# arkworks-rs/poly-commit

Measured on AMD Instinct MI355X. Metric: MSM G1-scalar-pairs/sec inside KZG commit+open (MarlinKZG10<Bls12_381> shape, hiding off), inputs HBM-resident (host-input blocking calls: value_trait_shaped), higher is better.
Workload: dtype u32 limbs (381-bit Fq / 255-bit Fr modular integer); 1 GPU; MarlinKZG10<bls12_381> commit+open, dense poly deg 2^24 per GPU, true SRS resident, hiding off (BASELINE metric sizes: 2^20 = configs[1], 2^24 = north-star target); curve=bls12_381, log_degree=24, inflight=2, srs_window_table=True, parallelism=1 GPU

## Files before the change

### __graft_entry__.py

```python
import os
import subprocess
import sys

ROOT = os.path.dirname(os.path.abspath(__file__))
for p in (ROOT, os.path.join(ROOT, "tests"), os.path.join(ROOT, "oracle")):
    if p not in sys.path:
        sys.path.insert(0, p)


def build():
    import importlib
    b = importlib.import_module("poly_commit_amd.build")
    b.build()
    subprocess.check_call(["make", "-s", "-C", os.path.join(ROOT, "oracle")])
    mb = os.path.join(ROOT, "tools", "microbench")
    src = mb + ".hip"
    deps = [src] + [os.path.join(ROOT, "poly_commit_amd", "csrc", f) for f in ("ec.hpp", "fp32.hpp", "curves.hpp")]
    deps = [d for d in deps if os.path.exists(d)]
    if not os.path.exists(mb) or any(os.path.getmtime(d) > os.path.getmtime(mb) for d in deps):
        subprocess.check_call(["hipcc", "--offload-arch=gfx950", "-O3", "-std=c++17", "-w", "-o", mb, src])
    import poly_commit_amd as pc
    pc.load_library()


def smoke():
    import numpy as np
    import oracle_lib as O
    import poly_commit_amd as pc

    if not os.path.exists(pc.library_path()):
        raise RuntimeError("libpc_hip.so missing -- run build() first (no CPU fallback exists)")
    ctx = pc.Context(0)
    curve, d = "bls12_381", 1 << 10
    powers = O.gen_bases(curve, d + 1)
    coeffs = O.f_to_mont(curve, 1, O.gen_scalars(curve, 0x5EED0001, d + 1))
    z = O.f_to_mont(curve, 1, O.gen_scalars(curve, 7, 1))[0]
    srs = ctx.upload_srs(curve, powers)
    comm, _ = srs.msm(coeffs, montgomery=True)
    q = ctx.witness_poly(curve, coeffs, z)
    proof, _ = srs.msm(q, montgomery=True)
    rc1, want_c = O.kzg_commit(curve, powers, coeffs)
    rc2, want_w = O.kzg_open(curve, powers, coeffs, z)
    assert rc1 == 0 and rc2 == 0
    assert (comm == want_c).all(), "commitment differs from the oracle"
    assert (proof == want_w).all(), "opening proof differs from the oracle"
    srs.precompute(min_pairs=1)
    assert (srs.msm(coeffs, montgomery=True)[0] == want_c).all(), "commitment (window table) differs from the oracle"
    assert (srs.msm(q, montgomery=True)[0] == want_w).all(), "opening proof (window table) differs from the oracle"
    rows = np.ascontiguousarray(coeffs[:1024].reshape(32, 32, 4))
    can = O.f_from_mont(curve, 1, np.ascontiguousarray(coeffs[:1024])).reshape(32, 32, 4)
    many, _ = srs.msm_many(rows, montgomery=True)
    for k in (0, 17, 31):
        assert (many[k] == O.msm_naive(curve, powers[:32], np.ascontiguousarray(can[k]))).all(), "msm_many differs from the oracle"
    mat = coeffs[:1024].reshape(4, 256, 4)
    assert (ctx.ntt_batch(curve, mat, 10) == O.ntt_batch(curve, mat, 10)).all(), "NTT differs from the oracle"
    srs.free()
    ctx.close()
    print("smoke ok: commit, open (table-free and window table), msm_many and NTT bit-identical to the oracle")


if __name__ == "__main__":
    build()
    if len(sys.argv) > 1 and sys.argv[1] == "smoke":
        smoke()
```

### poly_commit_amd/csrc/ec.hpp

```cpp
#pragma once
#include "fp32.hpp"

namespace pc {

template <class C>
struct AffD {
  typedef Fd<typename C::FqP> Fq;
  Fq x, y;
  static PC_HD AffD infinity() { AffD a; a.x = Fq::zero(); a.y = Fq::zero(); return a; }
  PC_HD bool is_inf() const { return x.is_zero() && y.is_zero(); }
  static PC_HD AffD load(const uint32_t* p) { AffD a; a.x = Fq::load(p); a.y = Fq::load(p + Fq::N); return a; }
  PC_HD void store(uint32_t* p) const { x.store(p); y.store(p + Fq::N); }
  PC_HD AffD neg_if(bool s) const { AffD a; a.x = x; a.y = s ? y.neg() : y; return a; }
};

template <class C>
struct XyzzD {
  typedef Fd<typename C::FqP> Fq;
  static constexpr int WORDS = 4 * Fq::N;
  Fq X, Y, ZZ, ZZZ;

  static PC_HD XyzzD infinity() { XyzzD r; r.X = Fq::zero(); r.Y = Fq::zero(); r.ZZ = Fq::zero(); r.ZZZ = Fq::zero(); return r; }
  PC_HD bool is_inf() const { return ZZ.is_zero(); }
  static PC_HD XyzzD from_affine(const AffD<C>& a) {
    XyzzD r;
    if (a.is_inf()) return infinity();
    r.X = a.x; r.Y = a.y; r.ZZ = Fq::one(); r.ZZZ = Fq::one(); return r;
  }
  static PC_HD XyzzD load(const uint32_t* p) {
    XyzzD r; r.X = Fq::load(p); r.Y = Fq::load(p + Fq::N); r.ZZ = Fq::load(p + 2 * Fq::N); r.ZZZ = Fq::load(p + 3 * Fq::N); return r;
  }
  PC_HD void store(uint32_t* p) const { X.store(p); Y.store(p + Fq::N); ZZ.store(p + 2 * Fq::N); ZZZ.store(p + 3 * Fq::N); }

  static PC_HD XyzzD dbl_affine(const AffD<C>& a) {
    if (a.is_inf() || a.y.is_zero()) return infinity();
    XyzzD r;
    Fq U = a.y.dbl(), V = U.sqr(), W = U.mul(V), S = a.x.mul(V);
    Fq xx = a.x.sqr(), M = xx.dbl().add(xx);
    r.X = M.sqr().sub(S.dbl());
    r.Y = M.mul_add_mul(S.sub(r.X), W.neg(), a.y);
    r.ZZ = V; r.ZZZ = W;
    return r;
  }
  PC_HD XyzzD dbl() const {
    if (is_inf() || Y.is_zero()) return infinity();
    XyzzD r;
    Fq U = Y.dbl(), V = U.sqr(), W = U.mul(V), S = X.mul(V);
    Fq xx = X.sqr(), M = xx.dbl().add(xx);
    r.X = M.sqr().sub(S.dbl());
    r.Y = M.mul_add_mul(S.sub(r.X), W.neg(), Y);
    r.ZZ = V.mul(ZZ); r.ZZZ = W.mul(ZZZ);
    return r;
  }
  PC_HD void add_affine(const AffD<C>& a) {
    if (a.is_inf()) return;
    if (is_inf()) { X = a.x; Y = a.y; ZZ = Fq::one(); ZZZ = Fq::one(); return; }
    Fq U2 = a.x.mul(ZZ), S2 = a.y.mul(ZZZ);
    Fq Pp = U2.sub(X), R = S2.sub(Y);
    if (Pp.is_zero()) {
      if (R.is_zero()) *this = dbl_affine(a); else *this = infinity();
      return;
    }
    Fq PP = Pp.sqr(), PPP = Pp.mul(PP), Q = X.mul(PP);
    Fq X3 = R.sqr().sub(PPP).sub(Q.dbl());
    Y = R.mul_add_mul(Q.sub(X3), Y.neg(), PPP);
    X = X3;
    ZZ = ZZ.mul(PP); ZZZ = ZZZ.mul(PPP);
  }
  PC_HD void add_affine_lz(const AffD<C>& a, bool negate) {
    if (a.y.is_zero()) { if (a.x.is_zero()) return; }
    const Fq ay = negate ? a.y.neg_lz_canonical() : a.y;
    if (is_inf()) { X = a.x; Y = ay; ZZ = Fq::one(); ZZZ = Fq::one(); return; }
    Fq U2 = a.x.mul_lz(ZZ), S2 = ay.mul_lz(ZZZ);
    Fq Pp = U2.sub_lz(X), R = S2.sub_lz(Y);
    if (Pp.is_zero_lz()) {
      XyzzD t = canonical();
      AffD<C> b; b.x = a.x; b.y = ay.canon();
      t.add_affine(b);
      *this = t;
      return;
    }
    Fq PP = Pp.sqr_lz(), PPP = Pp.mul_lz(PP), Q = X.mul_lz(PP);
    Fq X3 = R.sqr_lz().sub_lz(PPP).sub_lz(Q.dbl_lz());
    Y = R.mul_add_mul_lz(Q.sub_lz(X3), Y.neg_lz(), PPP);
    X = X3;
    ZZ = ZZ.mul_lz(PP); ZZZ = ZZZ.mul_lz(PPP);
  }
  PC_HD XyzzD canonical() const { XyzzD r; r.X = X.canon1(); r.Y = Y.canon1(); r.ZZ = ZZ.canon1(); r.ZZZ = ZZZ.canon1(); return r; }
  PC_HD void add(const XyzzD& o) {
    if (o.is_inf()) return;
    if (is_inf()) { *this = o; return; }
    Fq U1 = X.mul(o.ZZ), U2 = o.X.mul(ZZ), S1 = Y.mul(o.ZZZ), S2 = o.Y.mul(ZZZ);
    Fq Pp = U2.sub(U1), R = S2.sub(S1);
    if (Pp.is_zero()) {
      if (R.is_zero()) *this = dbl(); else *this = infinity();
      return;
    }
    Fq PP = Pp.sqr(), PPP = Pp.mul(PP), Q = U1.mul(PP);
    Fq X3 = R.sqr().sub(PPP).sub(Q.dbl());
    Y = R.mul_add_mul(Q.sub(X3), S1.neg(), PPP);
    X = X3;
    ZZ = ZZ.mul(o.ZZ).mul(PP); ZZZ = ZZZ.mul(o.ZZZ).mul(PPP);
  }
  PC_HD AffD<C> to_affine() const {
    if (is_inf()) return AffD<C>::infinity();
    Fq t = ZZ.mul(ZZZ).inv();
    AffD<C> a; a.x = X.mul(t.mul(ZZZ)); a.y = Y.mul(t.mul(ZZ)); return a;
  }
};


template <class C>
struct HalfPt {
  typedef Fd<typename C::FqP> Fq;
  Fq a, b;
  static PC_HD HalfPt of(const XyzzD<C>& p, bool odd) { HalfPt h; h.a = odd ? p.Y : p.X; h.b = odd ? p.ZZZ : p.ZZ; return h; }
};
template <class Fq>
PC_HD Fq fq_sel(bool c, const Fq& x, const Fq& y) {
  Fq r;
  PC_UNROLL for (int i = 0; i < Fq::N; i++) r.l[i] = c ? x.l[i] : y.l[i];
  return r;
}
template <class C>
struct HalfAdd {
  typedef Fd<typename C::FqP> Fq;
  Fq T1, D, DD, BB, T5, rc1, R6, X3;
  PC_HD bool p1(const HalfPt<C>& p, const HalfPt<C>& o) { T1 = p.a.mul(o.b); const Fq T2 = o.a.mul(p.b); D = T2.sub(T1); return D.is_zero(); }
  PC_HD Fq p2(const HalfPt<C>& p, const HalfPt<C>& o, bool odd) { DD = D.sqr(); BB = p.b.mul(o.b); T5 = D.mul(DD); return fq_sel(odd, DD, T5); }
  PC_HD Fq p3(bool odd, const Fq& recv) {
    rc1 = recv;
    R6 = fq_sel(odd, BB, T1).mul(fq_sel(odd, rc1, DD));
    X3 = rc1.sub(T5).sub(R6.dbl());
    return R6.sub(X3);
  }
  PC_HD void p4(HalfPt<C>& p, bool odd, const Fq& rc2) {
    const Fq R7 = fq_sel(odd, D, BB).mul_add_mul(fq_sel(odd, rc2, DD), fq_sel(odd, T1.neg(), Fq::zero()), fq_sel(odd, rc1, Fq::zero()));
    p.a = fq_sel(odd, R7, X3);
    p.b = fq_sel(odd, R6, R7);
  }
};

template <class C>
struct JacD {
  typedef Fd<typename C::FqP> Fq;
  Fq X, Y, Z;
  static PC_HD JacD infinity() { JacD r; r.X = Fq::one(); r.Y = Fq::one(); r.Z = Fq::zero(); return r; }
  PC_HD bool is_inf() const { return Z.is_zero(); }
  PC_HD JacD dbl() const {
    if (is_inf() || Y.is_zero()) return infinity();
    Fq A = X.sqr(), B = Y.sqr(), Cc = B.sqr();
    Fq t = X.add(B).sqr().sub(A).sub(Cc);
    Fq D = t.dbl(), E = A.dbl().add(A), F = E.sqr();
    JacD r;
    r.X = F.sub(D.dbl());
    r.Z = Y.mul(Z).dbl();
    r.Y = E.mul(D.sub(r.X)).sub(Cc.dbl().dbl().dbl());
    return r;
  }
  PC_HD void add_affine(const AffD<C>& a) {
    if (a.is_inf()) return;
    if (is_inf()) { X = a.x; Y = a.y; Z = Fq::one(); return; }
    Fq Z1Z1 = Z.sqr(), U2 = a.x.mul(Z1Z1), S2 = a.y.mul(Z).mul(Z1Z1);
    Fq H = U2.sub(X), rr = S2.sub(Y);
    if (H.is_zero()) {
      if (rr.is_zero()) *this = dbl(); else *this = infinity();
      return;
    }
    rr = rr.dbl();
    Fq HH = H.sqr(), I = HH.dbl().dbl(), J = H.mul(I), V = X.mul(I);
    Fq X3 = rr.sqr().sub(J).sub(V.dbl());
    Fq Y3 = rr.mul_add_mul(V.sub(X3), Y.dbl().neg(), J);
    Z = Z.add(H).sqr().sub(Z1Z1).sub(HH);
    X = X3; Y = Y3;
  }
  PC_HD AffD<C> to_affine() const {
    if (is_inf()) return AffD<C>::infinity();
    Fq zi = Z.inv(), zi2 = zi.sqr();
    AffD<C> a; a.x = X.mul(zi2); a.y = Y.mul(zi2).mul(zi); return a;
  }
};

template <class C>
struct JacBatchAffineBody {
  typedef Fd<typename C::FqP> Fq;
  static constexpr int FN = Fq::N, AW = 2 * FN;
  const uint32_t* jac;
  uint32_t* scratch;
  uint32_t* out;
  uint32_t n, K;
// ... 53 lines not shown
```

### poly_commit_amd/csrc/msm.hpp

```cpp
#pragma once
#include <stddef.h>
#include <stdint.h>
#include <algorithm>
#include <stdexcept>
#include <vector>
#include "ec.hpp"
#include "glv.hpp"
#include "host_tail.hpp"

#if defined(__HIP_DEVICE_COMPILE__)
#define PC_ARRIVED(PT, IDX)                                                                                             \
  do {                                                                                                                  \
    constexpr int PC_N_ = sizeof((PT).x.l) / 4;                                                                         \
    for (int pc_i_ = 0; pc_i_ < PC_N_; pc_i_ += 4) asm volatile("" ::"v"((PT).x.l[pc_i_]), "v"((PT).y.l[pc_i_]));     \
    asm volatile("" ::"v"(IDX));                                                                                        \
  } while (0)
#define PC_ARRIVED_WORD(W) asm volatile("" ::"v"(W))
#else
#define PC_ARRIVED(PT, IDX) ((void)0)
#define PC_ARRIVED_WORD(W) ((void)0)
#endif

#ifndef PC_ACC_DEBUG_IDX_MASK
#define PC_ACC_DEBUG_IDX_MASK 0x7fffffffu
// ... 106 lines not shown
        neg[h] = m[h][4] >> 31; m[h][4] &= 0x7fffffffu;
      }
    }
    PC_UNROLL for (int h = 0; h < 2; h++) {
      uint32_t carry = 0;
      const uint32_t ng = neg[h];
      for_each_window_limbs<5>(m[h], g.c, g.Wd / 2, [&](uint32_t w, uint32_t bits) {
        const uint32_t raw = bits + carry;
        carry = raw > half;
        const uint32_t mag = carry ? (2 * half - raw) : raw;
        if (mag) f((uint32_t)h, w, mag, carry ^ ng);
      });
    }
  }
}
template <class C>
struct GlvPresplitBody {
  typedef typename C::FrP FrP;
  MsmGeom g;
  const uint32_t* scalars;
  uint32_t* split;
  PC_HD void operator()(uint32_t i) const {
    uint32_t sub, j; g.split(i, sub, j);
    ScalarDigits<FrP> sd; sd.load(g.scalar_at(scalars, i, sub, j, FrP::N), g.from_mont);
    GlvHalves<C> hv; hv.split(sd.s);
    uint32_t* o = split + (size_t)i * GLV_SPLIT_WORDS;
    PC_UNROLL for (int h = 0; h < 2; h++) {
      PC_UNROLL for (int k = 0; k < 4; k++) o[5 * h + k] = hv.m[h][k];
      o[5 * h + 4] = hv.m[h][4] | (hv.neg[h] << 31);
    }
  }
};
template <class C, class Geo, class F>
PC_HD void for_each_signed_digit(const Geo& g, const uint32_t* scalar, F f) {
  if (g.glv) for_each_signed_digit_t<C, 1>(g, scalar, f); else for_each_signed_digit_t<C, 0>(g, scalar, f);
}

template <class C>
struct DigitsHistBody {
  typedef typename C::FrP FrP;
  MsmGeom g;
  const uint32_t* scalars;
  uint32_t* hist;
  PC_HD void operator()(uint32_t i) const {
    uint32_t sub, j; g.split(i, sub, j);
    for_each_signed_digit<C>(g, g.scalar_at(scalars, i, sub, j, FrP::N), [&](uint32_t h, uint32_t w, uint32_t mag, uint32_t) {
      atomic_inc_u32(hist + (size_t)g.key_window(w, sub, h) * g.nb_win + (mag - 1));
    });
  }
};

template <class C>
struct ScatterBody {
  typedef typename C::FrP FrP;
  MsmGeom g;
  const uint32_t* scalars;
  uint32_t* cursor;
  uint32_t* entries;
  PC_HD void operator()(uint32_t i) const {
    uint32_t sub, j; g.split(i, sub, j);
    for_each_signed_digit<C>(g, g.scalar_at(scalars, i, sub, j, FrP::N), [&](uint32_t h, uint32_t w, uint32_t mag, uint32_t neg) {
      const uint32_t pos = atomic_inc_u32(cursor + (size_t)g.key_window(w, sub, h) * g.nb_win + (mag - 1));
      entries[pos] = g.base_index(w, j) | (neg << 31);
    });
  }
};

PC_HD uint32_t find_bucket(const uint32_t* offs, uint32_t nb, uint32_t v) {
  uint32_t lo = 0, hi = nb;
  while (hi - lo > 1) {
    uint32_t mid = (lo + hi) >> 1;
    if (offs[mid] <= v) lo = mid; else hi = mid;
  }
  return lo;
}

PC_HD void partial_slot_range(const uint32_t* offs, uint32_t key, uint32_t T, uint32_t T2, uint32_t T2b, uint32_t level,
                              uint32_t& lo, uint32_t& hi) {
  lo = 2 * (offs[key] / T);
  hi = 2 * ((offs[key + 1] - 1) / T);
  for (uint32_t l = 2; l <= level; l++) { const uint32_t d = (l == 2) ? T2 : T2b; lo = 2 * (lo / d); hi = 2 * (hi / d); }
}

template <class C>
struct AccumulateBody {
  typedef XyzzD<C> Pt;
  static constexpr int AW = 2 * Fd<typename C::FqP>::N;
  MsmGeom g;
  const uint32_t* bases;
  const uint32_t* entries;
  const uint32_t* offsets;
  uint32_t* buckets;
  uint32_t* pkeys;
  uint32_t* ppts;
  static constexpr bool LAZY = Pt::Fq::LAZY_OK;
  static constexpr bool LAZY_STORE = LAZY && Pt::Fq::LAZY_STORE_OK;
  static PC_HD Pt store_form(const Pt& acc) { if constexpr (LAZY && !LAZY_STORE) return acc.canonical(); else return acc; }
  PC_HD void flush(const Pt& acc_lz, uint32_t k, bool complete, uint32_t t, bool first, uint32_t& k0, uint32_t& k1) const {
    const Pt& acc = acc_lz;
    if (complete) { acc.store(buckets + (size_t)k * Pt::WORDS); return; }
    uint32_t slot = first ? 2 * t : 2 * t + 1;
    acc.store(ppts + (size_t)slot * Pt::WORDS);
    if (first) k0 = k; else k1 = k;
  }
  PC_HD void chunk(uint32_t t, uint32_t& k0, uint32_t& k1, Pt& last) const {
    const uint32_t M = offsets[g.NB];
    const uint64_t s64 = (uint64_t)t * g.T;
    k0 = KEY_INVALID; k1 = KEY_INVALID;
    if (s64 < M) {
      const uint32_t s = (uint32_t)s64;
      const uint32_t e = (M - s > g.T) ? s + g.T : M;
      uint32_t k = find_bucket(offsets, g.NB, s);
      uint32_t run_lo = offsets[k], boundary = offsets[k + 1];
      uint32_t next_boundary = offsets[k + 2 <= g.NB ? k + 2 : g.NB];
      Pt acc = Pt::infinity();
      bool first = true;
      uint32_t val = entries[s];
      uint32_t nval = (s + 1 < e) ? entries[s + 1] : val;
      AffD<C> pt = AffD<C>::load(bases + (size_t)(val & PC_ACC_DEBUG_IDX_MASK) * g.pt_stride);
      for (uint32_t p = s; p < e; p++) {
        PC_ARRIVED(pt, nval);
        PC_ARRIVED_WORD(next_boundary);
        if (p == boundary) {
          flush(store_form(acc), k, run_lo >= s, t, first, k0, k1);
          first = false; acc = Pt::infinity();
          k++; run_lo = p; boundary = next_boundary;
          while (boundary <= p) { k++; boundary = offsets[k + 1]; }
        }
        const AffD<C> npt = AffD<C>::load(bases + (size_t)(nval & PC_ACC_DEBUG_IDX_MASK) * g.pt_stride);
        const uint32_t nnval = entries[p + 2 < e ? p + 2 : e - 1];
        next_boundary = offsets[k + 2 <= g.NB ? k + 2 : g.NB];
        if constexpr (LAZY) acc.add_affine_lz(pt, (val >> 31) != 0); else acc.add_affine(pt.neg_if(val >> 31));
        val = nval; nval = nnval; pt = npt;
      }
      acc = store_form(acc);
      flush(acc, k, run_lo >= s && boundary <= e, t, first, k0, k1);
      last = acc;
    }
  }
  PC_HD void operator()(uint32_t t) const {
    uint32_t k0, k1; Pt last;
    chunk(t, k0, k1, last);
    pkeys[2 * t] = k0; pkeys[2 * t + 1] = k1;
  }
};

template <class C>
struct SegReduceBody {
  static constexpr bool LATENCY_BOUND = true;
  typedef XyzzD<C> Pt;
  MsmGeom g;
  uint32_t level;
  uint32_t n_in;
  const uint32_t* in_keys; const uint32_t* in_pts;
  const uint32_t* offsets;
  uint32_t* buckets;
  uint32_t* out_keys; uint32_t* out_pts;
  PC_HD void flush(const Pt& acc, uint32_t key, uint32_t cs, uint32_t ce, uint32_t u, bool first, uint32_t& k0, uint32_t& k1) const {
    uint32_t lo, hi; partial_slot_range(offsets, key, g.T, g.T2, g.T2b, level, lo, hi);
    if (lo >= cs && hi < ce) { acc.store(buckets + (size_t)key * Pt::WORDS); return; }
    uint32_t slot = first ? 2 * u : 2 * u + 1;
    acc.store(out_pts + (size_t)slot * Pt::WORDS);
    if (first) k0 = key; else k1 = key;
  }
  PC_HD void operator()(uint32_t u) const {
    const uint32_t T2l = level == 1 ? g.T2 : g.T2b;
    const uint32_t cs = u * T2l;
    const uint32_t ce = (n_in - cs > T2l) ? cs + T2l : n_in;
    uint32_t k0 = KEY_INVALID, k1 = KEY_INVALID;
    uint32_t cur = KEY_INVALID; bool first = true;
    Pt acc = Pt::infinity();
    for (uint32_t p = cs; p < ce; p++) {
      uint32_t key = in_keys[p];
      if (key == KEY_INVALID) continue;
      if (key != cur) {
        if (cur != KEY_INVALID) { flush(acc, cur, cs, ce, u, first, k0, k1); first = false; }
        cur = key; acc = Pt::infinity();
      }
      acc.add(Pt::load(in_pts + (size_t)p * Pt::WORDS));
    }
    if (cur != KEY_INVALID) flush(acc, cur, cs, ce, u, first, k0, k1);
    out_keys[2 * u] = k0; out_keys[2 * u + 1] = k1;
  }
};

template <class C>
struct BucketLevelBody {
  static constexpr bool LATENCY_BOUND = true;
  typedef XyzzD<C> Pt;
  uint32_t K, weight_off, cnt, n_old;
  const uint32_t* x;
  const uint32_t* old_in;
  uint32_t* out;
  PC_HD void operator()(uint32_t lane) const {
    const uint32_t a = lane / cnt, gidx = lane % cnt;
    const size_t stride = (size_t)cnt * Pt::WORDS;
    if (a == 0) {
      const uint32_t* base = x + (size_t)gidx * K * Pt::WORDS;
      Pt run = Pt::infinity(), acc = Pt::infinity();
      Pt nxt = Pt::load(base + (size_t)(K - 1) * Pt::WORDS);
      for (uint32_t j = K; j-- > 0;) {
        const Pt cur = nxt;
        nxt = Pt::load(base + (size_t)(j > 0 ? j - 1 : 0) * Pt::WORDS);
        run.add(cur);
        if (j + weight_off > 0) acc.add(run);
      }
      run.store(out + (size_t)gidx * Pt::WORDS);
      acc.store(out + stride + (size_t)gidx * Pt::WORDS);
    } else {
      const uint32_t* base = old_in + (size_t)(a - 1) * cnt * K * Pt::WORDS + (size_t)gidx * K * Pt::WORDS;
      Pt acc = Pt::infinity();
      Pt nxt = Pt::load(base);
      for (uint32_t j = 0; j < K; j++) {
        const Pt cur = nxt;
        nxt = Pt::load(base + (size_t)(j + 1 < K ? j + 1 : j) * Pt::WORDS);
        acc.add(cur);
      }
      acc.store(out + (size_t)(1 + a) * stride + (size_t)gidx * Pt::WORDS);
    }
  }
// ... 603 lines not shown
```

### poly_commit_amd/csrc/msm_coop.hpp

```cpp
#pragma once
#include <hip/hip_runtime.h>
#include "msm.hpp"

namespace pc {

template <class C>
struct LdsPoints {
  typedef XyzzD<C> Pt;
  uint32_t* base; uint32_t lanes;
  __device__ __forceinline__ void put(uint32_t lane, const Pt& p) const {
    uint32_t w[Pt::WORDS]; p.store(w);
#pragma unroll
    for (int k = 0; k < Pt::WORDS; k++) base[k * lanes + lane] = w[k];
  }
  __device__ __forceinline__ Pt get(uint32_t lane) const {
    uint32_t w[Pt::WORDS];
#pragma unroll
    for (int k = 0; k < Pt::WORDS; k++) w[k] = base[k * lanes + lane];
    return Pt::load(w);
  }
};

template <class C>
__global__ void __launch_bounds__(256) k_bucket_level_coop(uint32_t K, uint32_t lgK, uint32_t weight_off, uint32_t cnt, uint32_t n_old,
// ... 33 lines not shown
template <class Fq>
__device__ __forceinline__ Fq lane_xchg(const Fq& v) {
  Fq r;
#pragma unroll
  for (int i = 0; i < Fq::N; i++) r.l[i] = (uint32_t)__builtin_amdgcn_mov_dpp((int)v.l[i], 0xB1, 0xF, 0xF, true);
  return r;
}

template <class C>
__device__ __forceinline__ void half_add(HalfPt<C>& p, const HalfPt<C>& o, bool odd) {
  typedef Fd<typename C::FqP> Fq;
  if (o.b.is_zero()) return;
  if (p.b.is_zero()) { p = o; return; }
  HalfAdd<C> h;
  const int dz = h.p1(p, o) ? 1 : 0, dz_nb = __builtin_amdgcn_mov_dpp(dz, 0xB1, 0xF, 0xF, true);
  const bool pz = odd ? dz_nb != 0 : dz != 0, rz = odd ? dz != 0 : dz_nb != 0;
  if (pz) {
    const Fq na = lane_xchg(p.a), nb = lane_xchg(p.b);
    XyzzD<C> f;
    f.X = fq_sel(odd, na, p.a); f.Y = fq_sel(odd, p.a, na); f.ZZ = fq_sel(odd, nb, p.b); f.ZZZ = fq_sel(odd, p.b, nb);
    p = HalfPt<C>::of(rz ? f.dbl() : XyzzD<C>::infinity(), odd);
    return;
  }
  const Fq rc1 = lane_xchg(h.p2(p, o, odd));
  const Fq rc2 = lane_xchg(h.p3(odd, rc1));
  h.p4(p, odd, rc2);
}

template <class C>
__global__ void __launch_bounds__(256) k_bucket_level_coop2(uint32_t K, uint32_t lgK, uint32_t weight_off, uint32_t cnt, uint32_t n_old,
                                                           const uint32_t* x, const uint32_t* old_in, uint32_t* out) {
  PC_LATENCY_KERNEL();
  typedef XyzzD<C> Pt;
  typedef Fd<typename C::FqP> Fq;
  constexpr int FN = Fq::N;
  extern __shared__ __attribute__((aligned(16))) uint32_t smem[];
  const uint32_t a = blockIdx.x / cnt, gidx = blockIdx.x % cnt, tid = threadIdx.x, l = tid >> 1, L = 2 * K;
  const bool odd = (tid & 1u) != 0;
  const uint32_t oa = odd ? FN : 0, ob = odd ? 3 * FN : 2 * FN;
  const size_t stride = (size_t)cnt * Pt::WORDS;
  const uint32_t nw = lgK + weight_off;
  const uint32_t* src = (a == 0) ? x + ((size_t)gidx * K + l) * Pt::WORDS
                                 : old_in + ((size_t)(a - 1) * cnt * K + (size_t)gidx * K + l) * Pt::WORDS;
  HalfPt<C> v; v.a = Fq::load(src + oa); v.b = Fq::load(src + ob);
  auto put = [&]() {
#pragma unroll
    for (int k = 0; k < FN; k++) { smem[k * L + tid] = v.a.l[k]; smem[(FN + k) * L + tid] = v.b.l[k]; }
  };
  auto get = [&](uint32_t t2) {
    HalfPt<C> r;
#pragma unroll
    for (int k = 0; k < FN; k++) { r.a.l[k] = smem[k * L + t2]; r.b.l[k] = smem[(FN + k) * L + t2]; }
    return r;
  };
  auto store = [&](uint32_t* dst) { v.a.store(dst + oa); v.b.store(dst + ob); };
  if (a == 0) {
    for (uint32_t d = 0; d < lgK; d++) {
      put();
      __syncthreads();
      const uint32_t low = l & ((2u << d) - 1u);
      if ((low & (low - 1u)) == 0 && low < (1u << d)) half_add<C>(v, get(tid + (2u << d)), odd);
      __syncthreads();
    }
    uint32_t* o = out + (size_t)gidx * Pt::WORDS;
    if (l == 0) { store(o); if (weight_off) store(o + (size_t)(1 + lgK) * stride); }
    else if ((l & (l - 1u)) == 0) { uint32_t b = 31 - __builtin_clz(l); store(o + (size_t)(1 + b) * stride); }
  } else {
    for (uint32_t d = K >> 1; d >= 1; d >>= 1) {
      put();
      __syncthreads();
      if (l < d) half_add<C>(v, get(tid + 2 * d), odd);
      __syncthreads();
    }
    if (l == 0) store(out + (size_t)(nw + a) * stride + (size_t)gidx * Pt::WORDS);
  }
}

#ifndef PC_ACC_WAVES_PER_EU
#define PC_ACC_WAVES_PER_EU 1
#endif
#ifndef PC_ACC_WAVES_N8
#define PC_ACC_WAVES_N8 1
#endif
template <class C> struct AccTune { static constexpr int WAVES = Fd<typename C::FqP>::N <= 8 ? PC_ACC_WAVES_N8 : PC_ACC_WAVES_PER_EU; };
#define PC_ACC_BOUNDS __launch_bounds__(256, AccTune<C>::WAVES)
template <class C>
__global__ void PC_ACC_BOUNDS k_accumulate(AccumulateBody<C> b, uint32_t lanes) {
  typedef XyzzD<C> Pt;
  __shared__ uint32_t xch[Pt::WORDS * 256];
  __shared__ uint32_t key_out[256], key_first[256], flags[256];
  const uint32_t tid = threadIdx.x, t = blockIdx.x * 256 + tid;
  const bool valid = t < lanes;
  uint32_t k0 = KEY_INVALID, k1 = KEY_INVALID;
  Pt V = Pt::infinity();
  if (valid) b.chunk(t, k0, k1, V);
  const uint32_t M = b.offsets[b.g.NB];
  const uint64_t s64 = (uint64_t)t * b.g.T;
  const uint32_t cs = s64 < M ? (uint32_t)s64 : M;
  const uint32_t ce = (M - cs > b.g.T) ? cs + b.g.T : M;
  const bool head_left = k0 != KEY_INVALID && b.offsets[k0] < cs;
  const bool head_right = k0 != KEY_INVALID && k1 == KEY_INVALID && b.offsets[k0 + 1] > ce;
  const bool transparent = head_left && head_right;
  const uint32_t okey = k1 != KEY_INVALID ? k1 : head_right ? k0 : KEY_INVALID;
  LdsPoints<C> lds{xch, 256};
  uint32_t fl = (okey == KEY_INVALID || !transparent) ? 1u : 0u;
  for (uint32_t d = 1; d < 256; d <<= 1) {
    const bool need = !(fl & 1u);
    if (!__syncthreads_or(need)) break;
    if (okey != KEY_INVALID) lds.put(tid, V);
    flags[tid] = fl;
    __syncthreads();
    if (need) {
      if (tid < d) fl = 3u;
      else { V.add(lds.get(tid - d)); fl = flags[tid - d]; }
    }
    __syncthreads();
  }
  key_out[tid] = okey; key_first[tid] = head_left ? k0 : KEY_INVALID; flags[tid] = fl;
  if (okey != KEY_INVALID) lds.put(tid, V);
  __syncthreads();
  const bool take = head_left && tid > 0 && key_out[tid - 1] == k0;
  const bool give = okey != KEY_INVALID && tid < 255 && key_first[tid + 1] == okey;
  if (transparent) {
    if (give) k0 = KEY_INVALID;
    else V.store(b.ppts + (size_t)(2 * t) * Pt::WORDS);
  } else {
    if (take) {
      uint32_t* slot = b.ppts + (size_t)(2 * t) * Pt::WORDS;
      Pt f = Pt::load(slot);
      f.add(lds.get(tid - 1));
      if (!(flags[tid - 1] & 2u) && !head_right) { f.store(b.buckets + (size_t)k0 * Pt::WORDS); k0 = KEY_INVALID; }
      else f.store(slot);
    }
    if (give) { if (k1 != KEY_INVALID) k1 = KEY_INVALID; else k0 = KEY_INVALID; }
  }
  if (valid) { b.pkeys[2 * t] = k0; b.pkeys[2 * t + 1] = k1; }
}

static constexpr uint32_t EDGE_REACH = 8;
template <class C>
__global__ void __launch_bounds__(64) k_accumulate_edges(AccumulateBody<C> b, uint32_t lanes) {
  PC_LATENCY_KERNEL();
  typedef XyzzD<C> Pt;
  const uint32_t k = blockIdx.x * 64 + threadIdx.x;
  const uint64_t t64 = (uint64_t)(k + 1) * 256;
  if (t64 >= lanes) return;
  const uint32_t t = (uint32_t)t64, a = t - 1;
  const uint32_t M = b.offsets[b.g.NB];
  uint32_t aslot = 2 * a + 1, key = b.pkeys[aslot];
  if (key == KEY_INVALID) {
    aslot = 2 * a; key = b.pkeys[aslot];
    if (key == KEY_INVALID || (uint64_t)b.offsets[key + 1] <= t64 * b.g.T) return;
  }
  uint32_t u = t;
  for (;; u++) {
    if (u >= lanes || u - t >= EDGE_REACH) return;
    const uint32_t ku = b.pkeys[2 * u];
    if (ku == key) break;
    if (ku != KEY_INVALID) return;
  }
  const uint64_t us = (uint64_t)u * b.g.T;
  const uint32_t ue = (M - (uint32_t)us > b.g.T) ? (uint32_t)us + b.g.T : M;
  uint32_t* slot = b.ppts + (size_t)(2 * u) * Pt::WORDS;
  Pt f = Pt::load(slot);
  f.add(Pt::load(b.ppts + (size_t)aslot * Pt::WORDS));
  b.pkeys[aslot] = KEY_INVALID;
  const uint64_t ws = (uint64_t)(a - 255u) * b.g.T;
// ... 24 lines not shown
```

Before: 481.3 million pairs/s.

## Accumulate BLS12-381 buckets in 30-bit-limb lazy Montgomery representation

Adds a 13x30-bit limb field type for BLS12-381 Fq with column-wise Montgomery multiplication whose carry headroom is planned at compile time. The bucket-accumulate kernel uses it for its running XYZZ sum, converting affine inputs on the fly and converting back to 32-bit limbs at flush. The aim is to cut carry-propagation work and reductions per field multiply via lazy bounds tracked by template parameters. It also raises the accumulate kernel's waves-per-EU bound to 2, trading register budget for occupancy, at the cost of conversion overhead and more limbs per multiply.

```diff
diff --git a/__graft_entry__.py b/__graft_entry__.py
--- a/__graft_entry__.py
+++ b/__graft_entry__.py
@@ -15,7 +15,7 @@
     subprocess.check_call(["make", "-s", "-C", os.path.join(ROOT, "oracle")])
     mb = os.path.join(ROOT, "tools", "microbench")
     src = mb + ".hip"
-    deps = [src] + [os.path.join(ROOT, "poly_commit_amd", "csrc", f) for f in ("ec.hpp", "fp32.hpp", "curves.hpp")]
+    deps = [src] + [os.path.join(ROOT, "poly_commit_amd", "csrc", f) for f in ("ec.hpp", "fp32.hpp", "fp30.hpp", "curves.hpp")]
     deps = [d for d in deps if os.path.exists(d)]
     if not os.path.exists(mb) or any(os.path.getmtime(d) > os.path.getmtime(mb) for d in deps):
         subprocess.check_call(["hipcc", "--offload-arch=gfx950", "-O3", "-std=c++17", "-w", "-o", mb, src])
diff --git a/poly_commit_amd/csrc/ec.hpp b/poly_commit_amd/csrc/ec.hpp
--- a/poly_commit_amd/csrc/ec.hpp
+++ b/poly_commit_amd/csrc/ec.hpp
@@ -1,5 +1,6 @@
 #pragma once
 #include "fp32.hpp"
+#include "fp30.hpp"
 
 namespace pc {
 
@@ -106,6 +107,44 @@
     if (is_inf()) return AffD<C>::infinity();
     Fq t = ZZ.mul(ZZZ).inv();
     AffD<C> a; a.x = X.mul(t.mul(ZZZ)); a.y = Y.mul(t.mul(ZZ)); return a;
+  }
+};
+
+
+struct XyzzR30 {
+  typedef pc_curve_bls12_381 C;
+  typedef Fd<C::FqP> F32;
+  typedef Fq30 Fq;
+  Fq X, Y, ZZ, ZZZ;
+
+  static PC_HD XyzzR30 infinity() { XyzzR30 r; r.X = Fq::zero(); r.Y = Fq::zero(); r.ZZ = Fq::zero(); r.ZZZ = Fq::zero(); return r; }
+  PC_HD bool is_inf() const { return ZZ.is_zero_exact(); }
+  PC_HD XyzzD<C> to32() const { XyzzD<C> r; r.X = X.to32(); r.Y = Y.to32(); r.ZZ = ZZ.to32(); r.ZZZ = ZZZ.to32(); return r; }
+  static PC_HD XyzzR30 from32(const XyzzD<C>& p) {
+    XyzzR30 r; r.X = Fq::from32(p.X); r.Y = Fq::from32(p.Y); r.ZZ = Fq::from32(p.ZZ).reduce(); r.ZZZ = Fq::from32(p.ZZZ).reduce(); return r;
+  }
+  PC_HD void add_affine(const AffD<C>& a, bool negate) {
+    if (a.y.is_zero()) { if (a.x.is_zero()) return; }
+    const F32 ay32 = negate ? a.y.neg_lz_canonical() : a.y;
+    const Fq ax = Fq::from32(a.x), ay = Fq::from32(ay32);
+    if (is_inf()) { X = ax; Y = ay; ZZ = Fq::one(); ZZZ = Fq::one(); return; }
+    const Fq U2 = Fq::mul<64, 2>(ax, ZZ), S2 = Fq::mul<64, 2>(ay, ZZZ);
+    const Fq Pp = Fq::sub<64>(U2, X), R = Fq::sub<64>(S2, Y);
+    if (Pp.is_zero_modp<66>()) {
+      if (R.is_zero_modp<66>()) { AffD<C> b; b.x = a.x; b.y = ay32.canon(); *this = from32(XyzzD<C>::dbl_affine(b)); }
+      else *this = infinity();
+      return;
+    }
+    const Fq PP = Fq::sqr<66>(Pp);
+    const Fq PPP = Fq::mul<66, 8>(Pp, PP), Q = Fq::mul<64, 8>(X, PP);
+    const Fq RR = Fq::sqr<66>(R);
+    const Fq X3 = Fq::sub_dbl<4>(Fq::sub<2>(RR, PPP), Q);
+    const Fq T = Fq::sub<14>(Q, X3), NY = Fq::neg<64>(Y);
+    Y = Fq::mul_add_mul<66, 16, 64, 2>(R, T, NY, PPP);
+    X = X3;
+    ZZ = Fq::mul<2, 8>(ZZ, PP); ZZZ = Fq::mul<2, 2>(ZZZ, PPP);
+    static_assert(Fq::mul_out(64 * 2) <= 2 && Fq::mul_out(66 * 66) <= 8 && Fq::mul_out(66 * 8) <= 2 && Fq::mul_out(64 * 8) <= 2, "classes of add_affine");
+    static_assert(Fq::mul_out(66 * 16 + 64 * 2) <= 64 && 8 + 2 + 4 <= 64 && Fq::mul_out(2 * 8) <= 2 && Fq::mul_out(2 * 2) <= 2, "the invariant closes");
   }
 };
 
diff --git a/poly_commit_amd/csrc/fp30.hpp b/poly_commit_amd/csrc/fp30.hpp
--- /dev/null
+++ b/poly_commit_amd/csrc/fp30.hpp
@@ -0,0 +1,338 @@
+#pragma once
+#include "fp32.hpp"
+
+#ifndef PC_ACC_R30
+#define PC_ACC_R30 1
+#endif
+
+namespace pc {
+
+struct Fq30Const {
+  typedef pc_bls12_381_fq P;
+  typedef unsigned __int128 u128;
+  static constexpr int N = 13;
+  static constexpr uint32_t MASK = (1u << 30) - 1;
+  struct L13 { uint32_t v[N]; };
+  struct W12 { uint32_t w[12]; };
+  static constexpr L13 recut_c(const uint32_t* w, int S) {
+    L13 r{};
+    for (int i = 0; i < N; i++) {
+      uint32_t v = 0;
+      for (int b = 0; b < 30; b++) {
+        const int src = 30 * i + b - S;
+        if (src >= 0 && src < 384) v |= ((w[src >> 5] >> (src & 31)) & 1u) << b;
+      }
+      r.v[i] = v;
+    }
+    return r;
+  }
+  static constexpr L13 kp(int V) {
+    uint32_t w[13] = {};
+    uint64_t c = 0;
+    for (int i = 0; i < 12; i++) { c += (uint64_t)P::MOD[i] * (uint32_t)V; w[i] = (uint32_t)c; c >>= 32; }
+    w[12] = (uint32_t)c;
+    L13 r{};
+    for (int i = 0; i < N; i++) {
+      uint32_t v = 0;
+      for (int b = 0; b < 30; b++) { const int src = 30 * i + b; if (src < 416) v |= ((w[src >> 5] >> (src & 31)) & 1u) << b; }
+      r.v[i] = v;
+    }
+    return r;
+  }
+  static constexpr W12 pow2_c(int S) {
+    W12 x{};
+    for (int i = 0; i < 12; i++) x.w[i] = P::ONE[i];
+    for (int s = 0; s < S; s++) {
+      uint32_t c = 0;
+      for (int i = 0; i < 12; i++) { const uint32_t t = x.w[i]; x.w[i] = (t << 1) | c; c = t >> 31; }
+      uint32_t d[12] = {}; uint64_t br = 0;
+      for (int i = 0; i < 12; i++) { const uint64_t t = (uint64_t)x.w[i] - P::MOD[i] - br; d[i] = (uint32_t)t; br = t >> 63; }
+      if (br == 0) for (int i = 0; i < 12; i++) x.w[i] = d[i];
+    }
+    return x;
+  }
+  enum { MUL = 0, SQR = 1, DUAL = 2 };
+  static constexpr uint64_t lmax(int V, int i) { return i < N - 1 ? (uint64_t)MASK : ((uint64_t)V * ((uint64_t)P::MOD[11] + 1)) >> 8; }
+  struct Plan { bool split[2 * N - 1][3]; bool ok; };
+  static constexpr Plan plan(int kind, int VA, int VB, int VC, int VD) {
+    Plan pl{};
+    pl.ok = lmax(VA, N - 1) <= MASK && lmax(VB, N - 1) <= MASK && lmax(VC, N - 1) <= MASK && lmax(VD, N - 1) <= MASK;
+    const u128 U64MAX = ~(uint64_t)0;
+    u128 carry = 0;
+    for (int k = 0; k < 2 * N - 1; k++) {
+      const int i0 = k > N - 1 ? k - (N - 1) : 0, i1 = k < N - 1 ? k : N - 1;
+      u128 g[3] = {0, 0, 0};
+      for (int i = i0; i <= i1; i++) {
+        const int j = k - i;
+        if (kind == SQR) { if (i < j) g[0] += (u128)lmax(VA, i) * (2 * lmax(VA, j)); else if (i == j) g[0] += (u128)lmax(VA, i) * lmax(VA, i); }
+        else { g[0] += (u128)lmax(VA, i) * lmax(VB, j); if (kind == DUAL) g[1] += (u128)lmax(VC, i) * lmax(VD, j); }
+        g[2] += (u128)MASK * kp(1).v[j];
+      }
+      u128 acc = carry, aside = 0;
+      for (int gi = 0; gi < 3; gi++) {
+        if (g[gi] == 0) continue;
+        if (acc + g[gi] > U64MAX) {
+          pl.split[k][gi] = true;
+          aside += acc >> 32; acc = 0xffffffffu;
+          if (acc + g[gi] > U64MAX) pl.ok = false;
+        }
+        acc += g[gi];
+      }
+      carry = (acc >> 30) + (aside << 2);
+      if (carry > U64MAX || aside > U64MAX) pl.ok = false;
+    }
+    if (carry > 0xffffffffu) pl.ok = false;
+    return pl;
+  }
+};
+
+struct Fq30 : Fq30Const {
+  typedef Fd<P> F32;
+  uint32_t l[N];
+
+  static constexpr L13 PL = kp(1);
+  static constexpr uint32_t INV30 = P::INV & MASK;
+  static constexpr uint32_t PINV30 = (0u - P::INV) & MASK;
+  static constexpr W12 ONE390 = pow2_c(6);
+  static constexpr L13 ONE30 = recut_c(ONE390.w, 0);
+  static_assert(((uint64_t)PL.v[0] * INV30 & MASK) == MASK, "INV30 = -p^-1 mod 2^30");
+  static_assert((uint64_t)630 * ((uint64_t)P::MOD[11] + 1) <= ((uint64_t)1 << 38), "p/R' < 1/630");
+  static constexpr int mul_out(int prod) { return prod / 630 + 2; }
+
+  static PC_HD Fq30 zero() { Fq30 r; PC_UNROLL for (int i = 0; i < N; i++) r.l[i] = 0; return r; }
+  static PC_HD Fq30 of(const L13& c) { Fq30 r; PC_UNROLL for (int i = 0; i < N; i++) r.l[i] = c.v[i]; return r; }
+  static PC_HD Fq30 one() { constexpr L13 c = ONE30; return of(c); }
+  PC_HD bool is_zero_exact() const { uint32_t a = 0; PC_UNROLL for (int i = 0; i < N; i++) a |= l[i]; return a == 0; }
+
+  static PC_HD Fq30 from32(const F32& w) {
+    Fq30 r;
+    r.l[0] = (w.l[0] << 6) & MASK;
+    PC_UNROLL for (int i = 1; i < N; i++) {
+      const int o = 30 * i - 6, j = o >> 5, s = o & 31;
+      const uint64_t two = (uint64_t)w.l[j] | (j + 1 < 12 ? (uint64_t)w.l[j + 1] << 32 : 0);
+      r.l[i] = (uint32_t)(two >> s) & MASK;
+    }
+    return r;
+  }
+  PC_HD F32 to32() const {
+    constexpr L13 Pl = PL;
+    const uint32_t k = (l[0] * INV30) & 63u;
+    uint32_t t[N]; uint64_t c = 0;
+    PC_UNROLL for (int i = 0; i < N - 1; i++) { c += (uint64_t)k * Pl.v[i] + l[i]; t[i] = (uint32_t)c & MASK; c >>= 30; }
+    t[N - 1] = l[N - 1] + k * Pl.v[N - 1] + (uint32_t)c;
+    F32 r;
+    PC_UNROLL for (int j = 0; j < 12; j++) {
+      const int o = 32 * j + 6, q = o / 30, s = o % 30;
+      const uint64_t two = (uint64_t)t[q] | ((uint64_t)t[q + 1] << 30);
+      r.l[j] = (uint32_t)(two >> s);
+    }
+    return r;
+  }
+  PC_HD Fq30 reduce() const { return mul<64, 1>(*this, one()); }
+
+  template <int V>
+  static PC_HD Fq30 sub(const Fq30& a, const Fq30& b) {
+    constexpr L13 K = kp(V);
+    Fq30 r; int32_t c = 0;
+    PC_UNROLL for (int i = 0; i < N - 1; i++) {
+      const int32_t t = (int32_t)(a.l[i] - b.l[i] + K.v[i]) + c;
+      r.l[i] = (uint32_t)t & MASK; c = t >> 30;
+    }
+    r.l[N - 1] = a.l[N - 1] - b.l[N - 1] + K.v[N - 1] + (uint32_t)c;
+    return r;
+  }
+  template <int V>
+  static PC_HD Fq30 sub_dbl(const Fq30& a, const Fq30& b) {
+    constexpr L13 K = kp(V);
+    Fq30 r; int32_t c = 0;
+    PC_UNROLL for (int i = 0; i < N - 1; i++) {
+      const int32_t t = (int32_t)(a.l[i] - 2u * b.l[i] + K.v[i]) + c;
+      r.l[i] = (uint32_t)t & MASK; c = t >> 30;
+    }
+    r.l[N - 1] = a.l[N - 1] - 2u * b.l[N - 1] + K.v[N - 1] + (uint32_t)c;
+    return r;
+  }
+  template <int V>
+  static PC_HD Fq30 neg(const Fq30& a) {
+    constexpr L13 K = kp(V);
+    Fq30 r; int32_t c = 0;
+    PC_UNROLL for (int i = 0; i < N - 1; i++) {
+      const int32_t t = (int32_t)(K.v[i] - a.l[i]) + c;
+      r.l[i] = (uint32_t)t & MASK; c = t >> 30;
+    }
+    r.l[N - 1] = K.v[N - 1] - a.l[N - 1] + (uint32_t)c;
+    return r;
+  }
+  template <int V>
+  PC_HD bool is_zero_modp() const {
+    const uint32_t q = (l[0] * PINV30) & MASK;
+    if (q > (uint32_t)V) return false;
+    constexpr L13 Pl = PL;
+    uint64_t c = 0; uint32_t diff = 0;
+    PC_UNROLL for (int i = 0; i < N - 1; i++) { c += (uint64_t)q * Pl.v[i]; diff |= l[i] ^ ((uint32_t)c & MASK); c >>= 30; }
+    c += (uint64_t)q * Pl.v[N - 1];
+    return diff == 0 && c == (uint64_t)l[N - 1];
+  }
+
+  template <int KIND, int VA, int VB, int VC, int VD>
+  struct PlanOf { static constexpr Plan value = plan(KIND, VA, VB, VC, VD); };
+
+#if defined(__HIP_DEVICE_COMPILE__)
+#define PC30_MAC1(A, B) "v_mad_u64_u32 %0, vcc, " A ", " B ", %0\n\t"
+#define PC30_MAC_FNS(NAME, YC)                                                                                          \
+  static __device__ __forceinline__ void NAME##1(uint64_t& acc, const uint32_t* x, const uint32_t* y) {                \
+    asm(PC30_MAC1("%1", "%2") : "+v"(acc) : "v"(x[0]), YC(y[0]) : "vcc");                                               \
+  }                                                                                                                     \
+  static __device__ __forceinline__ void NAME##2(uint64_t& acc, const uint32_t* x, const uint32_t* y) {                \
+    asm(PC30_MAC1("%1", "%2") PC30_MAC1("%3", "%4") : "+v"(acc) : "v"(x[0]), YC(y[0]), "v"(x[1]), YC(y[1]) : "vcc");    \
+  }                                                                                                                     \
+  static __device__ __forceinline__ void NAME##4(uint64_t& acc, const uint32_t* x, const uint32_t* y) {                \
+    asm(PC30_MAC1("%1", "%2") PC30_MAC1("%3", "%4") PC30_MAC1("%5", "%6") PC30_MAC1("%7", "%8")                         \
+        : "+v"(acc) : "v"(x[0]), YC(y[0]), "v"(x[1]), YC(y[1]), "v"(x[2]), YC(y[2]), "v"(x[3]), YC(y[3]) : "vcc");      \
+  }                                                                                                                     \
+  static __device__ __forceinline__ void NAME##8(uint64_t& acc, const uint32_t* x, const uint32_t* y) {                \
+    asm(PC30_MAC1("%1", "%2") PC30_MAC1("%3", "%4") PC30_MAC1("%5", "%6") PC30_MAC1("%7", "%8")                         \
+        PC30_MAC1("%9", "%10") PC30_MAC1("%11", "%12") PC30_MAC1("%13", "%14") PC30_MAC1("%15", "%16")                  \
+        : "+v"(acc)                                                                                                     \
+        : "v"(x[0]), YC(y[0]), "v"(x[1]), YC(y[1]), "v"(x[2]), YC(y[2]), "v"(x[3]), YC(y[3]),                           \
+          "v"(x[4]), YC(y[4]), "v"(x[5]), YC(y[5]), "v"(x[6]), YC(y[6]), "v"(x[7]), YC(y[7]) : "vcc");                  \
+  }
+  PC30_MAC_FNS(mac, PC_Y_VGPR)
+  PC30_MAC_FNS(macs, PC_Y_SGPR)
+  template <int CNT>
+  static __device__ __forceinline__ void mac_n(uint64_t& acc, const uint32_t* x, const uint32_t* y) {
+    if constexpr (CNT >= 8) { mac8(acc, x, y); mac_n<CNT - 8>(acc, x + 8, y + 8); }
+    else if constexpr (CNT >= 4) { mac4(acc, x, y); mac_n<CNT - 4>(acc, x + 4, y + 4); }
+    else if constexpr (CNT >= 2) { mac2(acc, x, y); mac_n<CNT - 2>(acc, x + 2, y + 2); }
+    else if constexpr (CNT == 1) mac1(acc, x, y);
+  }
+  template <int CNT>
+  static __device__ __forceinline__ void mac_ns(uint64_t& acc, const uint32_t* x, const uint32_t* y) {
+    if constexpr (CNT >= 8) { macs8(acc, x, y); mac_ns<CNT - 8>(acc, x + 8, y + 8); }
+    else if constexpr (CNT >= 4) { macs4(acc, x, y); mac_ns<CNT - 4>(acc, x + 4, y + 4); }
+    else if constexpr (CNT >= 2) { macs2(acc, x, y); mac_ns<CNT - 2>(acc, x + 2, y + 2); }
+    else if constexpr (CNT == 1) macs1(acc, x, y);
+  }
+#elif defined(PC_FQ30_HOST_COLUMNS)
+  template <int CNT> static inline void mac_n(uint64_t& acc, const uint32_t* x, const uint32_t* y) { for (int i = 0; i < CNT; i++) acc += (uint64_t)x[i] * y[i]; }
+  template <int CNT> static inline void mac_ns(uint64_t& acc, const uint32_t* x, const uint32_t* y) { mac_n<CNT>(acc, x, y); }
+  static inline void macs1(uint64_t& acc, const uint32_t* x, const uint32_t* y) { mac_n<1>(acc, x, y); }
+#endif
+#if defined(__HIP_DEVICE_COMPILE__) || defined(PC_FQ30_HOST_COLUMNS)
+  static PC_D void set_aside(uint64_t& acc, uint64_t& aside) { aside += acc >> 32; acc &= 0xffffffffu; }
+  template <int K>
+  static PC_D void prod_terms(const uint32_t* x_, const uint32_t* y_, uint64_t& acc) {
+    constexpr int I0 = K > N - 1 ? K - (N - 1) : 0, I1 = K < N - 1 ? K : N - 1, CNT = I1 - I0 + 1;
+    uint32_t x[CNT], y[CNT];
+    int c = 0;
+    PC_UNROLL for (int i = I0; i <= I1; i++) { x[c] = x_[i]; y[c] = y_[K - i]; c++; }
+    mac_n<CNT>(acc, x, y);
+  }
+  template <int K>
+  static PC_D void sq_terms(const uint32_t* a, const uint32_t* d, uint64_t& acc) {
+    constexpr int I0 = K > N - 1 ? K - (N - 1) : 0;
+    constexpr int NC = (K + 1) / 2 - I0 > 0 ? (K + 1) / 2 - I0 : 0, DG = (K & 1) ? 0 : 1, CNT = NC + DG;
+    uint32_t x[CNT], y[CNT];
+    int c = 0;
+    PC_UNROLL for (int i = I0; i < I0 + NC; i++) { x[c] = a[i]; y[c] = d[K - i]; c++; }
+    if constexpr (DG) { x[c] = a[K / 2]; y[c] = a[K / 2]; c++; }
+    mac_n<CNT>(acc, x, y);
+  }
+  template <int KIND, int VA, int VB, int VC, int VD, int K>
+  static PC_D void column(const uint32_t* a, const uint32_t* b, const uint32_t* c, const uint32_t* d, uint32_t* m,
+                                                uint32_t* t, uint64_t& acc) {
+    constexpr Plan pl = PlanOf<KIND, VA, VB, VC, VD>::value;
+    constexpr bool ANY = pl.split[K][0] || pl.split[K][1] || pl.split[K][2];
+    uint64_t aside = 0;
+    if constexpr (pl.split[K][0]) set_aside(acc, aside);
+    if constexpr (KIND == SQR) sq_terms<K>(a, b, acc); else prod_terms<K>(a, b, acc);
+    if constexpr (KIND == DUAL) {
+      if constexpr (pl.split[K][1]) set_aside(acc, aside);
+      prod_terms<K>(c, d, acc);
+    }
+    if constexpr (pl.split[K][2]) set_aside(acc, aside);
+    constexpr int I0 = K > N - 1 ? K - (N - 1) : 0, R1 = K < N ? K - 1 : N - 1, RC = R1 - I0 + 1;
+    if constexpr (RC > 0) {
+      constexpr L13 Pl = PL;
+      uint32_t x[RC], y[RC];
+      int n = 0;
+      PC_UNROLL for (int i = I0; i <= R1; i++) { x[n] = m[i]; y[n] = Pl.v[K - i]; n++; }
+      mac_ns<RC>(acc, x, y);
+    }
+    if constexpr (K < N) {
+      m[K] = ((uint32_t)acc * INV30) & MASK;
+      constexpr uint32_t p0c = kp(1).v[0];
+      const uint32_t p0 = p0c;
+      macs1(acc, &m[K], &p0);
+    } else {
+      t[K - N] = (uint32_t)acc & MASK;
+    }
+    acc >>= 30;
+    if constexpr (ANY) acc += aside << 2;
+    if constexpr (K + 1 < 2 * N - 1) column<KIND, VA, VB, VC, VD, K + 1>(a, b, c, d, m, t, acc);
+  }
+  template <int KIND, int VA, int VB, int VC, int VD>
+  static PC_D Fq30 mont_cols(const uint32_t* a, const uint32_t* b, const uint32_t* c, const uint32_t* d) {
+    uint32_t m[N], t[N];
+    uint64_t acc = 0;
+    column<KIND, VA, VB, VC, VD, 0>(a, b, c, d, m, t, acc);
+    t[N - 1] = (uint32_t)acc;
+    Fq30 r;
+    PC_UNROLL for (int i = 0; i < N; i++) r.l[i] = t[i];
+    return r;
+  }
+#endif
+#if !defined(__HIP_DEVICE_COMPILE__)
+  static inline Fq30 mont_rows_host(const Fq30& a, const Fq30& b, const Fq30* c, const Fq30* d) {
+    uint64_t t[N + 1];
+    for (int i = 0; i <= N; i++) t[i] = 0;
+    for (int i = 0; i < N; i++) {
+      for (int pass = 0; pass < (c ? 2 : 1); pass++) {
+        const Fq30& x = pass ? *c : a; const uint64_t yi = pass ? d->l[i] : b.l[i];
+        uint64_t cy = 0;
+        for (int j = 0; j < N; j++) { cy += t[j] + (uint64_t)x.l[j] * yi; t[j] = cy & MASK; cy >>= 30; }
+        t[N] += cy;
+      }
+      const uint64_t m = ((uint32_t)t[0] * INV30) & MASK;
+      uint64_t cy = (t[0] + m * PL.v[0]) >> 30;
+      for (int j = 1; j < N; j++) { cy += t[j] + m * PL.v[j]; t[j - 1] = cy & MASK; cy >>= 30; }
+      t[N - 1] = cy + t[N]; t[N] = 0;
+    }
+    Fq30 r;
+    for (int i = 0; i < N; i++) r.l[i] = (uint32_t)t[i];
+    return r;
+  }
+#endif
+
+  template <int VA, int VB>
+  static PC_HD Fq30 mul(const Fq30& a, const Fq30& b) {
+    static_assert(PlanOf<MUL, VA, VB, 0, 0>::value.ok, "a column of the product does not fit its accumulator");
+#if defined(__HIP_DEVICE_COMPILE__) || defined(PC_FQ30_HOST_COLUMNS)
+    return mont_cols<MUL, VA, VB, 0, 0>(a.l, b.l, nullptr, nullptr);
+#else
+    return mont_rows_host(a, b, nullptr, nullptr);
+#endif
+  }
+  template <int VA>
+  static PC_HD Fq30 sqr(const Fq30& a) {
+    static_assert(PlanOf<SQR, VA, VA, 0, 0>::value.ok, "a column of the squaring does not fit its accumulator");
+#if defined(__HIP_DEVICE_COMPILE__) || defined(PC_FQ30_HOST_COLUMNS)
+    uint32_t d[N];
+    PC_UNROLL for (int i = 0; i < N; i++) d[i] = a.l[i] << 1;
+    return mont_cols<SQR, VA, VA, 0, 0>(a.l, d, nullptr, nullptr);
+#else
+    return mont_rows_host(a, a, nullptr, nullptr);
+#endif
+  }
+  template <int VA, int VB, int VC, int VD>
+  static PC_HD Fq30 mul_add_mul(const Fq30& a, const Fq30& b, const Fq30& c, const Fq30& d) {
+    static_assert(PlanOf<DUAL, VA, VB, VC, VD>::value.ok, "a column of the fused pair does not fit its accumulator");
+#if defined(__HIP_DEVICE_COMPILE__) || defined(PC_FQ30_HOST_COLUMNS)
+    return mont_cols<DUAL, VA, VB, VC, VD>(a.l, b.l, c.l, d.l);
+#else
+    return mont_rows_host(a, b, &c, &d);
+#endif
+  }
+};
+
+}
diff --git a/poly_commit_amd/csrc/msm.hpp b/poly_commit_amd/csrc/msm.hpp
--- a/poly_commit_amd/csrc/msm.hpp
+++ b/poly_commit_amd/csrc/msm.hpp
@@ -212,9 +212,15 @@
   for (uint32_t l = 2; l <= level; l++) { const uint32_t d = (l == 2) ? T2 : T2b; lo = 2 * (lo / d); hi = 2 * (hi / d); }
 }
 
+template <class C> struct AccSum { static constexpr bool R30 = false; typedef XyzzD<C> type; };
+#if PC_ACC_R30
+template <> struct AccSum<pc_curve_bls12_381> { static constexpr bool R30 = true; typedef XyzzR30 type; };
+#endif
 template <class C>
 struct AccumulateBody {
   typedef XyzzD<C> Pt;
+  typedef typename AccSum<C>::type Sum;
+  static constexpr bool R30 = AccSum<C>::R30;
   static constexpr int AW = 2 * Fd<typename C::FqP>::N;
   MsmGeom g;
   const uint32_t* bases;
@@ -226,6 +232,7 @@
   static constexpr bool LAZY = Pt::Fq::LAZY_OK;
   static constexpr bool LAZY_STORE = LAZY && Pt::Fq::LAZY_STORE_OK;
   static PC_HD Pt store_form(const Pt& acc) { if constexpr (LAZY && !LAZY_STORE) return acc.canonical(); else return acc; }
+  static PC_HD Pt store_form(const XyzzR30& acc) { static_assert(!R30 || LAZY_STORE, "to32() hands over lazily reduced coordinates"); return acc.to32(); }
   PC_HD void flush(const Pt& acc_lz, uint32_t k, bool complete, uint32_t t, bool first, uint32_t& k0, uint32_t& k1) const {
     const Pt& acc = acc_lz;
     if (complete) { acc.store(buckets + (size_t)k * Pt::WORDS); return; }
@@ -243,7 +250,7 @@
       uint32_t k = find_bucket(offsets, g.NB, s);
       uint32_t run_lo = offsets[k], boundary = offsets[k + 1];
       uint32_t next_boundary = offsets[k + 2 <= g.NB ? k + 2 : g.NB];
-      Pt acc = Pt::infinity();
+      Sum acc = Sum::infinity();
       bool first = true;
       uint32_t val = entries[s];
       uint32_t nval = (s + 1 < e) ? entries[s + 1] : val;
@@ -253,19 +260,25 @@
         PC_ARRIVED_WORD(next_boundary);
         if (p == boundary) {
           flush(store_form(acc), k, run_lo >= s, t, first, k0, k1);
-          first = false; acc = Pt::infinity();
+          first = false; acc = Sum::infinity();
           k++; run_lo = p; boundary = next_boundary;
           while (boundary <= p) { k++; boundary = offsets[k + 1]; }
         }
         const AffD<C> npt = AffD<C>::load(bases + (size_t)(nval & PC_ACC_DEBUG_IDX_MASK) * g.pt_stride);
         const uint32_t nnval = entries[p + 2 < e ? p + 2 : e - 1];
         next_boundary = offsets[k + 2 <= g.NB ? k + 2 : g.NB];
-        if constexpr (LAZY) acc.add_affine_lz(pt, (val >> 31) != 0); else acc.add_affine(pt.neg_if(val >> 31));
+        if constexpr (R30) acc.add_affine(pt, (val >> 31) != 0);
+        else if constexpr (LAZY) acc.add_affine_lz(pt, (val >> 31) != 0); else acc.add_affine(pt.neg_if(val >> 31));
         val = nval; nval = nnval; pt = npt;
       }
-      acc = store_form(acc);
-      flush(acc, k, run_lo >= s && boundary <= e, t, first, k0, k1);
-      last = acc;
+      if constexpr (R30) {
+        last = store_form(acc);
+        flush(last, k, run_lo >= s && boundary <= e, t, first, k0, k1);
+      } else {
+        acc = store_form(acc);
+        flush(acc, k, run_lo >= s && boundary <= e, t, first, k0, k1);
+        last = acc;
+      }
     }
   }
   PC_HD void operator()(uint32_t t) const {
diff --git a/poly_commit_amd/csrc/msm_coop.hpp b/poly_commit_amd/csrc/msm_coop.hpp
--- a/poly_commit_amd/csrc/msm_coop.hpp
+++ b/poly_commit_amd/csrc/msm_coop.hpp
@@ -139,7 +139,7 @@
 #ifndef PC_ACC_WAVES_N8
 #define PC_ACC_WAVES_N8 1
 #endif
-template <class C> struct AccTune { static constexpr int WAVES = Fd<typename C::FqP>::N <= 8 ? PC_ACC_WAVES_N8 : PC_ACC_WAVES_PER_EU; };
+template <class C> struct AccTune { static constexpr int WAVES = Fd<typename C::FqP>::N <= 8 ? PC_ACC_WAVES_N8 : (AccSum<C>::R30 && PC_ACC_WAVES_PER_EU < 2) ? 2 : PC_ACC_WAVES_PER_EU; };
 #define PC_ACC_BOUNDS __launch_bounds__(256, AccTune<C>::WAVES)
 template <class C>
 __global__ void PC_ACC_BOUNDS k_accumulate(AccumulateBody<C> b, uint32_t lanes) {
```

After: 525.6 million pairs/s (median of 6 runs). +9.2%, better.
